# cover-vla/cover-vla

Measured on AMD Instinct MI355X. Metric: candidate actions scored/sec (whole node), OpenVLA-7B N=32, 224^2 RGB, higher is better.
Workload: dtype bf16; 1 GPU; OpenVLA-7B (DINOv2-L+SigLIP-So400m+Llama-2-7B) N=32 = 8 prompts x 4 samples per GPU, 7 action tokens, 1 224x224 RGB frame(s); CoVer verifier SigLIP2-L/16-384 + 3-member ensemble; random-init weights with decision margins (depth-scaled residual projections, unit-scale embeddings, log-normal gains on the action rows of the head: synth.openvla_state(peaked=True)); candidates_total=32, candidates_per_gpu=32, prompts_per_gpu=8, parallelism=candidate-sharded x1 (weak), own_kv=legacy

## Files before the change

### cover_vla_amd/_lib.py

```python
from __future__ import annotations

import ctypes as C
import os

import torch

_HERE = os.path.dirname(os.path.abspath(__file__))
LIB_PATH = os.environ.get("COVER_LIB_PATH") or os.path.join(_HERE, "libcover_hip.so")

c_p = C.c_void_p
c_ll = C.c_longlong
c_i = C.c_int
c_f = C.c_float


class CoverError(RuntimeError):
    pass


class GemmEpi(C.Structure):
    _fields_ = [("bias", c_p), ("residual", c_p), ("layer_scale", c_p), ("ld_residual", c_i), ("residual_f32", c_i),
                ("act", c_i), ("glu", c_i), ("out_f32", c_i), ("out_scale", c_f),
                ("norm_w", c_p), ("norm_out", c_p), ("ld_norm_out", c_i), ("norm_style", c_i), ("norm_w_offset", c_f),
                ("norm_eps", c_f), ("norm_b", c_p), ("w8", c_p), ("w8_scale", c_p), ("a8", c_p), ("a8_scale", c_p), ("ld_a8", c_i), ("ld_norm_out8", c_i),
                ("norm_out8", c_p), ("norm_out8_scale", c_p),
                ("a8_mx", c_p), ("out8", c_p), ("out8_mx", c_p), ("ld_out8", c_i), ("w8_klinear", c_i)]


class KvSegment(C.Structure):
    _fields_ = [("k", c_p), ("vt", c_p),
                ("k_slot_stride", c_ll), ("k_t_stride", c_ll), ("k_h_stride", c_ll),
                ("vt_slot_stride", c_ll), ("vt_h_stride", c_ll), ("vt_d_stride", c_ll),
                ("slot_of_batch", c_p), ("len_of_batch", c_p), ("vis_len", c_p),
                ("len", c_i), ("mask_mode", c_i), ("causal_offset", c_i), ("_pad", c_i)]


class AttnArgs(C.Structure):
    _fields_ = [("q", c_p), ("out", c_p),
                ("q_b_stride", c_ll), ("q_t_stride", c_ll), ("q_h_stride", c_ll),
                ("o_b_stride", c_ll), ("o_t_stride", c_ll), ("o_h_stride", c_ll),
                ("B", c_i), ("Tq", c_i), ("Hq", c_i), ("Hkv", c_i), ("D", c_i), ("scale", c_f),
                ("n_seg", c_i), ("_pad", c_i), ("seg", KvSegment * 3),
                ("state_in_o", c_p), ("state_in_ml", c_p), ("state_out_o", c_p), ("state_out_ml", c_p),
                ("out8", c_p), ("out8_mx", c_p), ("out8_rows", c_i), ("_pad2", c_i)]


class DecodeAttnArgs(C.Structure):
    _fields_ = [("qkv", c_p), ("ld_qkv", c_i), ("n_splits", c_i), ("partial", c_p), ("bias", c_p),
                ("N", c_i), ("H", c_i), ("D", c_i), ("scale", c_f),
                ("positions", c_p), ("cos_table", c_p), ("sin_table", c_p), ("n_pos", c_i), ("rope_mode", c_i),
                ("seg", KvSegment * 3), ("write_t", c_i), ("_pad", c_i), ("out", c_p), ("out_row_stride", c_ll)]


class OwnAttnArgs(C.Structure):
    _fields_ = [("qkv", c_p), ("ld_qkv", c_i), ("N", c_i), ("H", c_i), ("D", c_i), ("scale", c_f),
                ("positions", c_p), ("cos_table", c_p), ("sin_table", c_p), ("n_pos", c_i), ("rope_mode", c_i),
                ("k", c_p), ("v", c_p), ("k_scale", c_p), ("v_scale", c_p), ("fp8", c_i), ("t_cap", c_i),
                ("slot_stride", c_ll), ("slot_of_batch", c_p), ("write_t", c_i), ("_pad", c_i),
                ("state_o", c_p), ("state_ml", c_p)]


class RopeArgs(C.Structure):
    _fields_ = [("qkv", c_p), ("ld_qkv", c_i),
                ("B", c_i), ("T", c_i), ("Hq", c_i), ("Hkv", c_i), ("D", c_i),
                ("positions", c_p), ("cos_table", c_p), ("sin_table", c_p), ("n_pos", c_i),
                ("rope_mode", c_i),
                ("k_cache", c_p), ("k_slot_stride", c_ll), ("k_t_stride", c_ll), ("k_h_stride", c_ll),
# ... 297 lines not shown
```

### cover_vla_amd/csrc/attention.hip

```cpp
#include <stdlib.h>
#include <string.h>
#include "common.h"
#include "kernels.h"

struct SegDev {
    const bf16_t* k;
    const bf16_t* vt;
    long long k_slot, k_t, k_h, vt_slot, vt_h, vt_d;
    const int* slot_of_batch;
    const int* len_of_batch;
    const int* vis_len;
    int len, mode, causal_off;
};
struct AttnDev {
    const bf16_t* q;
    bf16_t* out;
    long long q_b, q_t, q_h, o_b, o_t, o_h;
    int B, Tq, Hq, Hkv, G, R;
    float scale_log2e;
    int n_seg;
    SegDev seg[3];
    const float* si_o; const float* si_ml;
    float* so_o; float* so_ml;
    uint8_t* o8; uint8_t* o8mx; int o8_rows;
    bool shared;
};

#ifdef COVER_AT_DEBUG
__device__ unsigned long long g_at_dbg[512 * 8];
extern "C" int cover_at_debug(unsigned long long* out) { return (int)hipMemcpyFromSymbol(out, HIP_SYMBOL(g_at_dbg), sizeof(g_at_dbg)); }
#define ATT(slot) do { if (threadIdx.x == 0) g_at_dbg[(((blockIdx.z * gridDim.y + blockIdx.y) * gridDim.x + blockIdx.x) & 511) * 8 + (slot)] = wall_clock64(); } while (0)
#else
#define ATT(slot) do { } while (0)
#endif
template <int D, bool KSPLIT, int NWS = 4, bool MXO = false>
__device__ __forceinline__ void attn_body(const AttnDev& a, int bx, int kvh, int b) {
    ATT(0);
    constexpr int KS = D / 32;
    constexpr int DB = D / 16;
    static_assert(!MXO || (KSPLIT && DB == 2 * NWS), "block-scaled output: two adjacent d blocks per wave");
    extern __shared__ __attribute__((aligned(16))) char smem[];
    const int lane = threadIdx.x & 63;
    const int w = __builtin_amdgcn_readfirstlane(threadIdx.x >> 6);
    const int nw = KSPLIT ? NWS : (int)(blockDim.x >> 6);
    const int tile = KSPLIT ? bx : bx * nw + w;
    const int r = lane & 15, g = lane >> 4;

    const int qi = tile * 16 + r;
    const bool q_ok = qi < a.R;
    const int qc = q_ok ? qi : 0;
    const int t = qc / a.G, gh = qc - t * a.G;
    const int h = kvh * a.G + gh;
    if (!KSPLIT && tile * 16 >= a.R) return;

    bf16x8 qf[KS];
    {
        const bf16_t* qp = a.q + (long long)b * a.q_b + (long long)t * a.q_t + (long long)h * a.q_h + g * 8;
#pragma unroll
        for (int ks = 0; ks < KS; ++ks) qf[ks] = as_bf16x8(*(const uint4*)(qp + ks * 32));
    }

#ifdef COVER_AT_DEBUG
    asm volatile("s_waitcnt vmcnt(0)" ::: "memory");
    ATT(1);
#endif
    float m_run = -INFINITY, l_run = 0.f;
    f32x4 oacc[DB];
#pragma unroll
    for (int db = 0; db < DB; ++db) oacc[db] = (f32x4){0.f, 0.f, 0.f, 0.f};
    const long long srow = ((long long)b * a.Tq + t) * a.Hq + h;
    if (a.si_o && q_ok && (!KSPLIT || w == 0)) {
        m_run = a.si_ml[srow * 2];
        l_run = a.si_ml[srow * 2 + 1];
        const float* so = a.si_o + srow * D + 4 * g;
#pragma unroll
        for (int db = 0; db < DB; ++db) {
            const float4 v = *(const float4*)(so + db * 16);
            oacc[db] = (f32x4){v.x * l_run, v.y * l_run, v.z * l_run, v.w * l_run};
        }
    }

    int t_hi = (tile * 16 + 15) / a.G;
    t_hi = t_hi < a.Tq ? t_hi : a.Tq - 1;

    int tile_counter = 0;
    for (int si = 0; si < a.n_seg; ++si) {
        const SegDev& sg = a.seg[si];
        const int slot = sg.slot_of_batch ? sg.slot_of_batch[b] : b;
        const int len = sg.len_of_batch ? sg.len_of_batch[b] : sg.len;
        int kend = len;
        if (sg.mode == COVER_MASK_CAUSAL) kend = min(kend, t_hi + sg.causal_off + 1);
        int vis = len;
        if (sg.mode == COVER_MASK_CAUSAL) vis = min(len, t + sg.causal_off + 1);
        else if (sg.mode == COVER_MASK_VISLEN) vis = min(len, sg.vis_len[t]);
        const bf16_t* kb = sg.k + (long long)slot * sg.k_slot + (long long)kvh * sg.k_h + g * 8;
        const bf16_t* vb = sg.vt + (long long)slot * sg.vt_slot + (long long)kvh * sg.vt_h + (long long)r * sg.vt_d + g * 8;

        for (int t0 = 0; t0 < kend; t0 += 32, ++tile_counter) {
            if (KSPLIT && (tile_counter & (nw - 1)) != w) continue;
            int key0 = t0 + 8 * (r >> 2) + (r & 3);
            int key1 = key0 + 4;
            key0 = key0 < len ? key0 : len - 1;
            key1 = key1 < len ? key1 : len - 1;
            const bf16_t* k0p = kb + (long long)key0 * sg.k_t;
            const bf16_t* k1p = kb + (long long)key1 * sg.k_t;
            const bf16_t* vp = vb + t0;
            uint4 kr0[KS], kr1[KS];
#pragma unroll
            for (int ks = 0; ks < KS; ++ks) {
                kr0[ks] = *(const uint4*)(k0p + ks * 32);
                kr1[ks] = *(const uint4*)(k1p + ks * 32);
            }
            constexpr bool V_EARLY = (D <= 128) || KSPLIT;
            uint4 vr[V_EARLY ? DB : 1];
            if (V_EARLY) {
#pragma unroll
                for (int db = 0; db < DB; ++db) vr[db] = *(const uint4*)(vp + (long long)(db * 16) * sg.vt_d);
            }
#ifdef COVER_AT_DEBUG
            if (tile_counter == 0) { asm volatile("s_waitcnt vmcnt(0)" ::: "memory"); ATT(2); }
#endif
            f32x4 s0 = (f32x4){0.f, 0.f, 0.f, 0.f}, s1 = s0;
#pragma unroll
            for (int ks = 0; ks < KS; ++ks) {
                s0 = __builtin_amdgcn_mfma_f32_16x16x32_bf16(as_bf16x8(kr0[ks]), qf[ks], s0, 0, 0, 0);
                s1 = __builtin_amdgcn_mfma_f32_16x16x32_bf16(as_bf16x8(kr1[ks]), qf[ks], s1, 0, 0, 0);
            }
            float sc[8];
            float tmax = -INFINITY;
#pragma unroll
            for (int e = 0; e < 8; ++e) {
                const float v = (e < 4 ? s0[e] : s1[e - 4]) * a.scale_log2e;
                const int key = t0 + 8 * g + e;
                sc[e] = (key < vis) ? v : -INFINITY;
                tmax = fmaxf(tmax, sc[e]);
            }
            tmax = fmaxf(tmax, __shfl_xor(tmax, 16));
            tmax = fmaxf(tmax, __shfl_xor(tmax, 32));
            const float m_new = fmaxf(m_run, tmax);
            float alpha = 1.f, psum = 0.f;
            float p[8];
            if (m_new == -INFINITY) {
#pragma unroll
                for (int e = 0; e < 8; ++e) p[e] = 0.f;
            } else {
                alpha = exp2f(m_run - m_new);
#pragma unroll
                for (int e = 0; e < 8; ++e) {
                    p[e] = exp2f(sc[e] - m_new);
                    psum += p[e];
                }
            }
            psum += __shfl_xor(psum, 16);
            psum += __shfl_xor(psum, 32);
            l_run = l_run * alpha + psum;
            m_run = m_new;
            uint4 pp;
            pp.x = pack_bf2(p[0], p[1]);
            pp.y = pack_bf2(p[2], p[3]);
            pp.z = pack_bf2(p[4], p[5]);
            pp.w = pack_bf2(p[6], p[7]);
            const bf16x8 pf = as_bf16x8(pp);
#pragma unroll
            for (int db = 0; db < DB; ++db) {
                const bf16x8 vf = as_bf16x8(V_EARLY ? vr[V_EARLY ? db : 0] : *(const uint4*)(vp + (long long)(db * 16) * sg.vt_d));
                f32x4 o = oacc[db];
                o[0] *= alpha; o[1] *= alpha; o[2] *= alpha; o[3] *= alpha;
                oacc[db] = __builtin_amdgcn_mfma_f32_16x16x32_bf16(vf, pf, o, 0, 0, 0);
            }
        }
    }

    ATT(3);
    int db_first = 0, db_step = 1;
    if (KSPLIT) {
        float* so = (float*)smem;
        constexpr int OW = DB * 4 * 64;
        float* sm = so + NWS * OW;
        float* sl = sm + NWS * 16;
#pragma unroll
        for (int db = 0; db < DB; ++db)
#pragma unroll
            for (int e = 0; e < 4; ++e) so[w * OW + (db * 4 + e) * 64 + lane] = oacc[db][e];
        if (g == 0) {
            sm[w * 16 + r] = m_run;
            sl[w * 16 + r] = l_run;
        }
        __syncthreads();
        float mi[NWS], li[NWS], f[NWS];
#pragma unroll
        for (int i = 0; i < NWS; ++i) {
            mi[i] = sm[i * 16 + r];
            li[i] = sl[i * 16 + r];
        }
        float mx = -INFINITY;
#pragma unroll
        for (int i = 0; i < NWS; ++i) mx = fmaxf(mx, mi[i]);
        float lt = 0.f;
// ... 315 lines not shown
            const float is = 1.0f / scl;
            const int col = h * (int)a.o_h + 32 * j;
#pragma unroll
            for (int k = 0; k < 2; ++k) {
                int pk = __builtin_amdgcn_cvt_pk_fp8_f32(v[k * 4] * is, v[k * 4 + 1] * is, 0, false);
                pk = __builtin_amdgcn_cvt_pk_fp8_f32(v[k * 4 + 2] * is, v[k * 4 + 3] * is, pk, true);
                *(uint32_t*)(a.o8 + ro + col + k * 16 + 4 * g) = (uint32_t)pk;
            }
            if (g == 0) a.o8mx[((size_t)(col >> 7) * a.o8_rows + (size_t)(ro / a.o_t)) * 4 + ((col >> 5) & 3)] = (uint8_t)((__builtin_bit_cast(uint32_t, scl) >> 23) & 0xffu);
        }
        ATT(5);
        return;
    }
    if (a.so_o) {
        if (g == 0) {
            a.so_ml[srow * 2] = m_run;
            a.so_ml[srow * 2 + 1] = l_run;
        }
        float* so = a.so_o + srow * D + 4 * g;
#pragma unroll
        for (int db = 0; db < DB; ++db) *(float4*)(so + db * 16) = make_float4(oacc[db][0] * inv, oacc[db][1] * inv, oacc[db][2] * inv, oacc[db][3] * inv);
        return;
    }
    bf16_t* op = a.out + (long long)b * a.o_b + (long long)t * a.o_t + (long long)h * a.o_h + 4 * g;
#pragma unroll
    for (int db = 0; db < DB; ++db) {
        uint2 v;
        v.x = pack_bf2(oacc[db][0] * inv, oacc[db][1] * inv);
        v.y = pack_bf2(oacc[db][2] * inv, oacc[db][3] * inv);
        *(uint2*)(op + db * 16) = v;
    }
    ATT(5);
}
template <int D, bool KSPLIT, int NWS = 4, bool MXO = false>
__global__ __launch_bounds__((KSPLIT && D > 128) ? 64 * NWS : 512) void attn_kernel(AttnDev a) {
    attn_body<D, KSPLIT, NWS, MXO>(a, blockIdx.x, blockIdx.y, blockIdx.z);
}
template <int D>
__global__ __launch_bounds__(512) void attn_kernel_dual(AttnDev a0, AttnDev a1, int tiles0, int n0, int tiles1) {
    int idx = blockIdx.x;
    if (idx < n0) {
        attn_body<D, true>(a0, idx % tiles0, blockIdx.y, idx / tiles0);
    } else {
        idx -= n0;
        attn_body<D, true>(a1, idx % tiles1, blockIdx.y, idx / tiles1);
    }
}

struct AttnEnv {
    bool shared_off, pair_off, has_ks_max;
    long long ks_max, nw8_max;
};
static const AttnEnv& attn_env() {
    static const AttnEnv e = [] {
        AttnEnv v;
        const char* sh = getenv("COVER_ATTN_SHARED");
        const char* pr = getenv("COVER_ATTN_PAIR");
        const char* mx = getenv("COVER_ATTN_KSPLIT_MAX");
        const char* n8 = getenv("COVER_ATTN_NW8_MAX");
        v.shared_off = sh && sh[0] == '0';
        v.pair_off = pr && pr[0] == '0';
        v.has_ks_max = mx != nullptr;
        v.ks_max = mx ? atoll(mx) : 1023;
        v.nw8_max = n8 ? atoll(n8) : 0;
        return v;
    }();
    return e;
}
static long long attn_qtiles(const cover_attn_args* x) {
    const int G = x->Hq / x->Hkv;
    return (long long)((x->Tq * G + 15) / 16) * x->Hkv * x->B;
}
static long long attn_ks_max(const cover_attn_args* x) {
    const AttnEnv& e = attn_env();
    return (x->state_in_o != nullptr && !e.has_ks_max && x->D <= 128) ? 4095 : e.ks_max;
}
static bool attn_shared_ok(const cover_attn_args* x) {
    if (attn_env().shared_off) return false;
    if (x->D != 128 || x->Hq != x->Hkv || x->Tq < 48 || x->n_seg < 1 || x->n_seg > 3) return false;
    for (int i = 0; i < x->n_seg; ++i)
        if (x->seg[i].mask_mode != COVER_MASK_LEN) return false;
    return (long long)((x->Tq + 63) / 64) * x->Hq * x->B >= 128;
}

bool attention_mx_ok(const cover_attn_args* x) {
    if (x->D != 128 || x->Hq != x->Hkv || x->Hkv <= 0 || x->state_out_o != nullptr || x->B <= 0 || x->Tq <= 0) return false;
    if (x->o_h_stride != 128 || x->o_t_stride != (long long)x->Hq * 128 || (x->o_b_stride % x->o_t_stride) != 0) return false;
    return attn_qtiles(x) <= attn_ks_max(x) || attn_shared_ok(x);
}

struct AttnPlan {
    int form, mxo, nw;
    dim3 grid;
    size_t lds;
};
static hipError_t attn_decide(const cover_attn_args* x, AttnPlan& p) {
    p.form = -1; p.mxo = 0; p.nw = 0; p.grid = dim3(0, 0, 0); p.lds = 0;
    const int G = x->Hq / x->Hkv, R = x->Tq * G;
    if (x->B <= 0 || R <= 0) return hipSuccess;
    const int D = x->D;
    if (D != 64 && D != 96 && D != 128 && D != 256) return hipErrorInvalidValue;
    const bool o8 = x->out8 != nullptr && x->out8_mx != nullptr;
    const int tiles = (R + 15) / 16;
    const long long qtiles = (long long)tiles * x->Hkv * x->B;
    const long long ks_max = attn_ks_max(x);
    p.mxo = o8 ? 1 : 0;
    if (attn_shared_ok(x)) {
        p.form = 3; p.nw = 4;
        p.grid = dim3((x->Tq + 63) / 64, x->Hq, x->B);
        return hipSuccess;
    }
    if (o8) {
        if (D != 128 || qtiles > ks_max) return hipErrorInvalidValue;
        p.form = 1; p.nw = 4;
    } else if (qtiles <= ks_max) {
        p.nw = (qtiles <= attn_env().nw8_max && D <= 128) ? 8 : 4;
        p.form = p.nw == 8 ? 2 : 1;
    } else {
        p.form = 0;
        p.nw = tiles >= 4 ? 4 : tiles;
        p.grid = dim3((tiles + p.nw - 1) / p.nw, x->Hkv, x->B);
        return hipSuccess;
    }
    p.grid = dim3(tiles, x->Hkv, x->B);
    p.lds = (size_t)(p.nw * (D / 16) * 4 * 64 + 2 * p.nw * 16) * sizeof(float);
    return hipSuccess;
}
static bool attn_pair_dual(const cover_attn_args* x0, const cover_attn_args* x1) {
    const AttnEnv& e = attn_env();
    const bool o8 = (x0->out8 && x0->out8_mx) || (x1->out8 && x1->out8_mx);
    return x0->D == x1->D && x0->Hkv == x1->Hkv && x0->B > 0 && x1->B > 0 && x0->Tq > 0 && x1->Tq > 0 && attn_qtiles(x0) <= e.ks_max &&
           attn_qtiles(x1) <= e.ks_max && (x0->D == 64 || x0->D == 96 || x0->D == 128) && !o8 && !e.pair_off;
}

static bool off16(const void* p) { return ((uintptr_t)p & 15) != 0; }
static hipError_t build_attn_dev(const cover_attn_args* x, AttnDev& a) {
    if (x->n_seg < 1 || x->n_seg > 3 || x->Hkv <= 0 || x->Hq % x->Hkv != 0) return hipErrorInvalidValue;
    a.q = (const bf16_t*)x->q;
    a.out = (bf16_t*)x->out;
    a.q_b = x->q_b_stride; a.q_t = x->q_t_stride; a.q_h = x->q_h_stride;
    a.o_b = x->o_b_stride; a.o_t = x->o_t_stride; a.o_h = x->o_h_stride;
    if (off16(a.q) || ((a.q_b | a.q_t | a.q_h) & 7)) return hipErrorInvalidValue;
    if (((uintptr_t)a.out & 7) || ((a.o_b | a.o_t | a.o_h) & 3)) return hipErrorInvalidValue;
    a.B = x->B; a.Tq = x->Tq; a.Hq = x->Hq; a.Hkv = x->Hkv;
    a.G = x->Hq / x->Hkv;
    a.R = x->Tq * a.G;
    a.scale_log2e = x->scale * 1.4426950408889634f;
    a.n_seg = x->n_seg;
    a.si_o = x->state_in_o; a.si_ml = x->state_in_ml; a.so_o = x->state_out_o; a.so_ml = x->state_out_ml;
    if ((a.si_o == nullptr) != (a.si_ml == nullptr) || (a.so_o == nullptr) != (a.so_ml == nullptr)) return hipErrorInvalidValue;
    if (off16(a.si_o) || off16(a.so_o) || ((uintptr_t)a.si_ml & 7) || ((uintptr_t)a.so_ml & 7)) return hipErrorInvalidValue;
    a.o8 = (uint8_t*)x->out8; a.o8mx = (uint8_t*)x->out8_mx; a.o8_rows = x->out8_rows;
    if (!a.o8 || !a.o8mx) { a.o8 = nullptr; a.o8mx = nullptr; }
    if (a.o8 && !attention_mx_ok(x)) return hipErrorInvalidValue;
    a.shared = attn_shared_ok(x);
    for (int i = 0; i < x->n_seg; ++i) {
        const cover_kv_segment& s = x->seg[i];
        SegDev& d = a.seg[i];
        d.k = (const bf16_t*)s.k; d.vt = (const bf16_t*)s.vt;
        d.k_slot = s.k_slot_stride; d.k_t = s.k_t_stride; d.k_h = s.k_h_stride;
        d.vt_slot = s.vt_slot_stride; d.vt_h = s.vt_h_stride; d.vt_d = s.vt_d_stride;
        d.slot_of_batch = s.slot_of_batch; d.len_of_batch = s.len_of_batch; d.vis_len = s.vis_len;
        d.len = s.len; d.mode = s.mask_mode; d.causal_off = s.causal_offset;
        if (d.mode == COVER_MASK_VISLEN && d.vis_len == nullptr) return hipErrorInvalidValue;
        if (off16(d.k) || off16(d.vt) || ((d.k_slot | d.k_t | d.k_h | d.vt_slot | d.vt_h | d.vt_d) & 7)) return hipErrorInvalidValue;
    }
    return hipSuccess;
}

hipError_t attention_plan(const cover_attn_args* x, int* plan) {
    AttnDev a;
    AttnPlan p;
    hipError_t e = build_attn_dev(x, a);
    if (e == hipSuccess) e = attn_decide(x, p);
    if (e != hipSuccess) return e;
    plan[0] = p.form; plan[1] = p.mxo; plan[2] = (int)(p.grid.x * p.grid.y * p.grid.z); plan[3] = p.nw;
    return hipSuccess;
}
hipError_t attention_pair_plan(const cover_attn_args* x0, const cover_attn_args* x1, int* dual) {
    AttnDev a;
    AttnPlan p;
    hipError_t e = build_attn_dev(x0, a);
    if (e == hipSuccess) e = attn_decide(x0, p);
    if (e == hipSuccess) e = build_attn_dev(x1, a);
    if (e == hipSuccess) e = attn_decide(x1, p);
    if (e != hipSuccess) return e;
    *dual = attn_pair_dual(x0, x1) ? 1 : 0;
    return hipSuccess;
}

template <int D>
static void launch_d(const AttnDev& a, const AttnPlan& p, hipStream_t st) {
    const dim3 block(64 * p.nw);
    if (p.form == 3) {
        if (p.mxo) hipLaunchKernelGGL((attn_shared_k<true>), p.grid, block, 0, st, a);
        else hipLaunchKernelGGL((attn_shared_k<false>), p.grid, block, 0, st, a);
    } else if (p.form == 1 && p.mxo) {
        if constexpr (D == 128) hipLaunchKernelGGL((attn_kernel<D, true, 4, true>), p.grid, block, p.lds, st, a);
    } else if (p.form == 2) {
        if constexpr (D <= 128) hipLaunchKernelGGL((attn_kernel<D, true, 8>), p.grid, block, p.lds, st, a);
    } else if (p.form == 1) {
        hipLaunchKernelGGL((attn_kernel<D, true, 4>), p.grid, block, p.lds, st, a);
    } else {
        hipLaunchKernelGGL((attn_kernel<D, false>), p.grid, block, 0, st, a);
    }
}
static hipError_t launch_planned(const cover_attn_args* x, const AttnDev& a, const AttnPlan& p, hipStream_t st) {
    if (p.form < 0) return hipSuccess;
    const int pid = prof_enabled() ? prof_open(st, 2, 0.0) : -1;
    switch (x->D) {
        case 64: launch_d<64>(a, p, st); break;
        case 96: launch_d<96>(a, p, st); break;
        case 128: launch_d<128>(a, p, st); break;
        default: launch_d<256>(a, p, st); break;
    }
    const hipError_t e = hipGetLastError();
    prof_close(st, pid);
    return e;
}

hipError_t launch_attention_bf16(const cover_attn_args* x, hipStream_t st) {
    AttnDev a;
    AttnPlan p;
    hipError_t e = build_attn_dev(x, a);
    if (e == hipSuccess) e = attn_decide(x, p);
    if (e != hipSuccess) return e;
    return launch_planned(x, a, p, st);
// ... 33 lines not shown
```

### cover_vla_amd/csrc/capi.hip

```cpp
#include <hip/hip_runtime.h>
#include <stdio.h>
#include <stdlib.h>
#include <string.h>
#include <string>
#include "kernels.h"

static thread_local std::string g_err;
static int fail(int code, const char* what, hipError_t e = hipSuccess) {
    char buf[512];
    if (e != hipSuccess) snprintf(buf, sizeof buf, "%s: %s", what, hipGetErrorString(e));
    else snprintf(buf, sizeof buf, "%s", what);
    g_err = buf;
    return code;
}
#define HIPCHK(call, what)                                  \
    do {                                                    \
        hipError_t _e = (call);                             \
        if (_e != hipSuccess) return fail(_e == hipErrorInvalidValue ? COVER_EINVAL : COVER_EHIP, what, _e); \
    } while (0)
#define ST(s) ((hipStream_t)(s))

extern "C" {

int cover_abi_version(void) { return COVER_ABI_VERSION; }
// ... 426 lines not shown
    size_t skb = 0;
    {
        const int ns[4] = {3 * HD, d->dim, d->mlp_p, d->dim};
        const int ks[4] = {d->dim, HD, d->dim, d->mlp_p};
        for (int i = 0; i < 4; ++i) {
            size_t b = gemm_workspace_bytes((int)R, ns[i], ks[i]);
            skb = b > skb ? b : skb;
        }
    }
    p = cc.take(skb); if (sk) *sk = p;
    if (sk_bytes) *sk_bytes = skb;
    return cc.off + 256;
}
size_t cover_vit_workspace_bytes(const cover_vit_desc* d, int n_seq, int T) {
    int tcap;
    return vit_ws(d, n_seq, T, nullptr, nullptr, nullptr, nullptr, nullptr, nullptr, nullptr, nullptr, &tcap);
}

__global__ void zero_u32_k(unsigned* __restrict__ p, size_t n) {
    for (size_t i = (size_t)blockIdx.x * blockDim.x + threadIdx.x; i < n; i += (size_t)gridDim.x * blockDim.x) p[i] = 0u;
}
int cover_vit_forward(const cover_vit_desc* d, void* x, int n_seq, int T, void* attn_out, cover_workspace ws, int variant,
                      void* stream) {
    if (!d || !x || !d->layers_host) return fail(COVER_EINVAL, "cover_vit_forward: null pointer");
    if (d->last_attn_only && !attn_out) return fail(COVER_EINVAL, "cover_vit_forward: last_attn_only needs attn_out");
    hipStream_t st = ST(stream);
    Carver c{(char*)ws.ptr, ws.bytes, 0};
    void *h, *qkv, *attn, *mlp, *vt, *sk;
    size_t skb;
    int tcap;
    const size_t need = vit_ws(d, n_seq, T, &c, &h, &qkv, &attn, &mlp, &vt, &sk, &skb, &tcap);
    if (!ws.ptr || ws.bytes < need) return fail(COVER_EWORKSPACE, "cover_vit_forward: workspace too small");
    const int R = n_seq * T, dim = d->dim, H = d->heads, Dp = d->head_dim_p, HD = H * Dp;
    if (tcap != T) {
        const size_t words = (size_t)n_seq * HD * tcap / 2;
        hipLaunchKernelGGL(zero_u32_k, dim3((unsigned)((words + 1023) / 1024 < 2048 ? (words + 1023) / 1024 : 2048)), dim3(256), 0, st, (unsigned*)vt, words);
        HIPCHK(hipGetLastError(), "zero vt");
    }

    HIPCHK(launch_layernorm_bf16((const bf16_t*)x, dim, d->layers_host[0].ln1_w, d->layers_host[0].ln1_b, (bf16_t*)h, dim, R, dim, d->ln_eps, st), "vit ln1");
    for (int l = 0; l < d->n_layers; ++l) {
        const cover_vit_layer& L = d->layers_host[l];
        cover_gemm_epi e;
        memset(&e, 0, sizeof e);
        e.out_scale = 1.0f;
        e.bias = L.qkv_b;
        HIPCHK(launch_gemm_bf16((const bf16_t*)h, dim, (const bf16_t*)L.qkv_w, qkv, 3 * HD, R, 3 * HD, dim, &e, (float*)sk, skb, variant, st), "vit qkv");
        cover_rope_args ra;
        memset(&ra, 0, sizeof ra);
        ra.qkv = qkv; ra.ld_qkv = 3 * HD; ra.B = n_seq; ra.T = T; ra.Hq = H; ra.Hkv = H; ra.D = Dp; ra.rope_mode = 0;
        ra.vt_cache = vt; ra.vt_slot_stride = (long long)HD * tcap; ra.vt_h_stride = (long long)Dp * tcap; ra.vt_d_stride = tcap;
        HIPCHK(launch_rope_kv_write(&ra, st), "vit v-transpose");
        cover_attn_args aa;
        memset(&aa, 0, sizeof aa);
        aa.q = qkv; aa.q_b_stride = (long long)T * 3 * HD; aa.q_t_stride = 3 * HD; aa.q_h_stride = Dp;
        aa.out = attn; aa.o_b_stride = (long long)T * HD; aa.o_t_stride = HD; aa.o_h_stride = Dp;
        aa.B = n_seq; aa.Tq = T; aa.Hq = H; aa.Hkv = H; aa.D = Dp; aa.scale = d->attn_scale; aa.n_seg = 1;
        aa.seg[0].k = (const bf16_t*)qkv + HD; aa.seg[0].k_slot_stride = (long long)T * 3 * HD; aa.seg[0].k_t_stride = 3 * HD; aa.seg[0].k_h_stride = Dp;
        aa.seg[0].vt = vt; aa.seg[0].vt_slot_stride = (long long)HD * tcap; aa.seg[0].vt_h_stride = (long long)Dp * tcap; aa.seg[0].vt_d_stride = tcap;
        aa.seg[0].len = T; aa.seg[0].mask_mode = COVER_MASK_LEN;
        HIPCHK(launch_attention_bf16(&aa, st), "vit attention");
        const bool last_attn = d->last_attn_only && l == d->n_layers - 1;
        memset(&e, 0, sizeof e);
        e.out_scale = 1.0f;
        e.bias = L.proj_b;
        if (last_attn) {
            HIPCHK(launch_gemm_bf16((const bf16_t*)attn, HD, (const bf16_t*)L.proj_w, attn_out, dim, R, dim, HD, &e, (float*)sk, skb, variant, st), "vit proj (tap)");
            break;
        }
        e.residual = x; e.ld_residual = dim; e.layer_scale = L.ls1;
        e.norm_w = L.ln2_w; e.norm_b = L.ln2_b; e.norm_out = h; e.ld_norm_out = dim; e.norm_style = 2; e.norm_eps = d->ln_eps;
        HIPCHK(launch_gemm_bf16((const bf16_t*)attn, HD, (const bf16_t*)L.proj_w, x, dim, R, dim, HD, &e, (float*)sk, skb, variant, st), "vit proj (+ln2)");
        memset(&e, 0, sizeof e);
        e.out_scale = 1.0f;
        e.bias = L.fc1_b; e.act = d->act;
        HIPCHK(launch_gemm_bf16((const bf16_t*)h, dim, (const bf16_t*)L.fc1_w, mlp, d->mlp_p, R, d->mlp_p, dim, &e, (float*)sk, skb, variant, st), "vit fc1");
        memset(&e, 0, sizeof e);
        e.out_scale = 1.0f;
        e.bias = L.fc2_b; e.residual = x; e.ld_residual = dim; e.layer_scale = L.ls2;
        if (l + 1 < d->n_layers) {
            const cover_vit_layer& Ln = d->layers_host[l + 1];
            e.norm_w = Ln.ln1_w; e.norm_b = Ln.ln1_b; e.norm_out = h; e.ld_norm_out = dim; e.norm_style = 2; e.norm_eps = d->ln_eps;
        }
        HIPCHK(launch_gemm_bf16((const bf16_t*)mlp, d->mlp_p, (const bf16_t*)L.fc2_w, x, dim, R, dim, d->mlp_p, &e, (float*)sk, skb, variant, st), "vit fc2 (+next ln1)");
    }
    return COVER_OK;
}

static size_t dec_ws(const cover_dec_desc* d, int rows, Carver* c, void** h, void** qkv, void** attn, void** mlp, void** sk,
                     size_t* sk_bytes, void** st_o = nullptr, void** st_ml = nullptr, void** q8 = nullptr, void** q8s = nullptr, void** q8mx = nullptr) {
    Carver tmp{nullptr, 0, 0};
    Carver& cc = c ? *c : tmp;
    const int nqkv = (d->Hq + 2 * d->Hkv) * d->D;
// ... 336 lines not shown
```

### cover_vla_amd/ops.py

```python
from __future__ import annotations

import ctypes as C
import math
from dataclasses import dataclass
from typing import Optional, Sequence, Union

import numpy as np
import torch

from . import _lib as L

ACT = {"none": 0, "gelu_tanh": 1, "gelu_erf": 2, "silu": 3, "relu": 4}
MASK_LEN, MASK_CAUSAL, MASK_VISLEN = 0, 1, 2


def _stream() -> int:
    return torch.cuda.current_stream().cuda_stream


def _ptr(t: Optional[torch.Tensor]) -> Optional[int]:
    return None if t is None else t.data_ptr()


def _chk_dev(*ts):
# ... 136 lines not shown
    torch.cuda.synchronize()
    buf = (C.c_ulonglong * 16)()
    L.check(L.lib().cover_gemm_probe(buf), "gemm_probe")
    w0, w1, w2, w3, c0, c1, nk = (int(buf[i]) for i in range(7))
    e4, e5, e6 = (int(buf[i]) for i in (12, 13, 14))
    loop_us = (w2 - w1) * 0.01
    staged = w2 <= e4 <= e5 <= e6 <= w3
    return dict(prologue_us=(w1 - w0) * 0.01, loop_us=loop_us, epilogue_us=(w3 - w2) * 0.01, k_tiles=nk,
                cycles_per_k_tile=(c1 - c0) / max(nk, 1), clock_ghz=(c1 - c0) / max(loop_us, 1e-9) / 1e3,
                epilogue_split_us=[(e4 - w2) * 0.01, (e5 - e4) * 0.01, (e6 - e5) * 0.01, (w3 - e6) * 0.01] if staged else None)


def gemm_plan_counts(reset: bool = False) -> list:
    n = 32
    buf = (C.c_longlong * n)()
    L.lib().cover_gemm_plan_counts(buf, n, 1 if reset else 0)
    return list(buf)


@dataclass
class Segment:
    k: torch.Tensor
    vt: torch.Tensor
    k_strides: Sequence[int]
    vt_strides: Sequence[int]
    length: int = 0
    len_of_batch: Optional[torch.Tensor] = None
    slot_of_batch: Optional[torch.Tensor] = None
    mask: int = MASK_LEN
    causal_offset: int = 0
    vis_len: Optional[torch.Tensor] = None
    k_offset: int = 0
    vt_offset: int = 0


def fill_segment(s: L.KvSegment, seg: Segment) -> None:
    s.k = seg.k.data_ptr() + 2 * seg.k_offset
    s.vt = seg.vt.data_ptr() + 2 * seg.vt_offset
    s.k_slot_stride, s.k_t_stride, s.k_h_stride = seg.k_strides
    s.vt_slot_stride, s.vt_h_stride, s.vt_d_stride = seg.vt_strides
    s.slot_of_batch = _ptr(seg.slot_of_batch)
    s.len_of_batch = _ptr(seg.len_of_batch)
    s.vis_len = _ptr(seg.vis_len)
    s.len = seg.length
    s.mask_mode = seg.mask
    s.causal_offset = seg.causal_offset


def attention_args(q: torch.Tensor, q_strides: Sequence[int], out: Optional[torch.Tensor], o_strides: Sequence[int], B: int, Tq: int,
                   Hq: int, Hkv: int, D: int, scale: float, segments: Sequence[Segment], state_in=None, state_out=None, out8=None) -> "L.AttnArgs":
    _chk_dev(q, out)
    a = L.AttnArgs()
    a._keep = (q, out, out8, state_in, state_out, list(segments))
    a.q, a.out = q.data_ptr(), _ptr(out)
    if out8 is not None:
        _chk_dev(out8[0], out8[1])
        assert out8[0].dtype == torch.uint8 and out8[1].dtype == torch.uint8 and out8[1].is_contiguous() and out8[0].is_contiguous()
        a.out8, a.out8_mx, a.out8_rows = out8[0].data_ptr(), out8[1].data_ptr(), out8[0].shape[0]
    if state_in is not None:
        a.state_in_o, a.state_in_ml = state_in[0].data_ptr(), state_in[1].data_ptr()
    if state_out is not None:
        a.state_out_o, a.state_out_ml = state_out[0].data_ptr(), state_out[1].data_ptr()
    a.q_b_stride, a.q_t_stride, a.q_h_stride = q_strides
    a.o_b_stride, a.o_t_stride, a.o_h_stride = o_strides
    a.B, a.Tq, a.Hq, a.Hkv, a.D, a.scale = B, Tq, Hq, Hkv, D, scale
    a.n_seg = len(segments)
    for i, sg in enumerate(segments[:3]):
        fill_segment(a.seg[i], sg)
    return a
# ... 997 lines not shown
```

### include/cover_hip.h

```cpp
#ifndef COVER_HIP_H
#define COVER_HIP_H
#include <stddef.h>
#include <stdint.h>

#ifdef __cplusplus
extern "C" {
#endif

#define COVER_ABI_VERSION 1

enum cover_status { COVER_OK = 0, COVER_EINVAL = -1, COVER_EHIP = -2, COVER_EWORKSPACE = -3, COVER_EUNSUPPORTED = -4 };
enum cover_act { COVER_ACT_NONE = 0, COVER_ACT_GELU_TANH = 1, COVER_ACT_GELU_ERF = 2, COVER_ACT_SILU = 3, COVER_ACT_RELU = 4 };

int cover_abi_version(void);
const char* cover_last_error(void);
int cover_device_info(int dev, int* n_cu, size_t* total_mem, char* name, int name_len);

typedef struct cover_gemm_epi {
    const float* bias;
    const void* residual;
    const float* layer_scale;
    int ld_residual;
    int residual_f32;
    int act;
// ... 25 lines not shown
size_t cover_packed_weight_bytes(int N, int K);
int cover_packed_k(int K);
int cover_pack_weight_bf16(const void* W, int ldw, int N, int K, void* Wp, int glu_interleave, void* stream);

size_t cover_packed_weight_fp8_bytes(int N, int K);
int cover_quantize_rows_fp8(const void* W, int ldw, int N, int K, float* scales, void* Wdq, void* stream);
int cover_pack_weight_fp8(const void* Wdq, int ldw, const float* scales, int N, int K, void* Wq, float* scales_packed,
                          int glu_interleave, void* stream);

int cover_quantize_act_fp8(const void* X, int ldx, int M, int K, void* out8, int ld8, float* scales, void* stream);
int cover_quantize_act_fp8_mx(const void* X, int ldx, int M, int K, void* out8, int ld8, void* mx, void* stream);
int cover_pack_weight_fp8_klinear(const void* Wdq, int ldw, const float* scales, int N, int K, void* Wq, float* scales_packed, void* stream);

size_t cover_gemm_workspace_bytes(int M, int N, int K);
int cover_gemm_bf16(const void* A, int lda, const void* Wp, void* C, int ldc, int M, int N, int K,
                    const cover_gemm_epi* epi, void* splitk_ws, size_t splitk_ws_bytes, int variant, void* stream);
int cover_gemm_plan_counts(long long* counts, int n, int reset);
int cover_gemm_plan(const void* A, int lda, const void* Wp, void* C, int ldc, int M, int N, int K,
                    const cover_gemm_epi* epi, void* splitk_ws, size_t splitk_ws_bytes, int variant, int plan[6]);
int cover_gemm_probe(unsigned long long* out);

enum cover_mask_mode { COVER_MASK_LEN = 0, COVER_MASK_CAUSAL = 1, COVER_MASK_VISLEN = 2 };
typedef struct cover_kv_segment {
    const void* k;
    const void* vt;
    long long k_slot_stride, k_t_stride, k_h_stride;
    long long vt_slot_stride, vt_h_stride, vt_d_stride;
    const int* slot_of_batch;
    const int* len_of_batch;
    const int* vis_len;
    int len;
    int mask_mode;
    int causal_offset;
    int _pad;
} cover_kv_segment;

typedef struct cover_attn_args {
    const void* q;
    void* out;
    long long q_b_stride, q_t_stride, q_h_stride;
    long long o_b_stride, o_t_stride, o_h_stride;
    int B, Tq, Hq, Hkv, D;
    float scale;
    int n_seg;
    int _pad;
    cover_kv_segment seg[3];
    const float* state_in_o; const float* state_in_ml;
    float* state_out_o; float* state_out_ml;
    void* out8; void* out8_mx;
    int out8_rows; int _pad2;
} cover_attn_args;
int cover_attention_bf16(const cover_attn_args* args, void* stream);
int cover_attention_plan(const cover_attn_args* args, int plan[4]);
int cover_attention_bf16_pair(const cover_attn_args* a0, const cover_attn_args* a1, void* stream);
int cover_attention_pair_plan(const cover_attn_args* a0, const cover_attn_args* a1, int* dual);

typedef struct cover_decode_attn_args {
    const void* qkv; int ld_qkv;
    int n_splits;
    const float* partial; const float* bias;
    int N, H, D;
    float scale;
    const int* positions; const float* cos_table; const float* sin_table; int n_pos; int rope_mode;
    cover_kv_segment seg[3];
    int write_t; int _pad;
    void* out; long long out_row_stride;
} cover_decode_attn_args;
// ... 270 lines not shown
    const float* logprobs;
    long long lp_n_stride, lp_t_stride;
    const int64_t* tokens;
    long long tok_n_stride, tok_t_stride;
    long long pad_token_id;
    int N, steps, group_size, top_m;
    float beta; int length_normalize;
    float* prior_out;
    float* combined_out;
    float* group_mean_out;
    int* result_out;
    float* best_out;
    int* ranked_out;
} cover_prior_select_args;
int cover_prior_select(const cover_prior_select_args* args, void* stream);

typedef struct cover_workspace { void* ptr; size_t bytes; } cover_workspace;

typedef struct cover_vit_layer {
    const float *ln1_w, *ln1_b, *ln2_w, *ln2_b;
    const void* qkv_w; const float* qkv_b;
    const void* proj_w; const float* proj_b;
    const void* fc1_w; const float* fc1_b;
    const void* fc2_w; const float* fc2_b;
    const float *ls1, *ls2;
} cover_vit_layer;
typedef struct cover_vit_desc {
    int dim, heads, head_dim_p, mlp_p, n_layers, act;
    float ln_eps, attn_scale;
    const cover_vit_layer* layers_host;
    int last_attn_only;
    int _pad;
} cover_vit_desc;
size_t cover_vit_workspace_bytes(const cover_vit_desc* d, int n_seq, int T);
int cover_vit_forward(const cover_vit_desc* d, void* x, int n_seq, int T, void* attn_out, cover_workspace ws,
                      int gemm_variant, void* stream);

typedef struct cover_dec_layer {
    const float* in_norm_w; const float* post_norm_w;
    const void* qkv_w; const float* qkv_b;
    const void* o_w;
    const void* gate_up_w;
    const void* down_w;
    void* k_cache; void* vt_cache;
    const void* qkv_w8; const float* qkv_s; const void* o_w8; const float* o_s;
    const void* gate_up_w8; const float* gate_up_s; const void* down_w8; const float* down_s;
    int down_klinear;
    int o_klinear;
} cover_dec_layer;
typedef struct cover_dec_desc {
    int dim, Hq, Hkv, D, mlp, n_layers, act;
    int norm_style;
    float norm_eps, norm_w_offset, attn_scale;
    int rope_mode; int n_pos; int _pad;
    const float* cos_table; const float* sin_table;
    const float* final_norm_w;
    const cover_dec_layer* layers_host;
} cover_dec_desc;
typedef struct cover_dec_group {
    int B, T;
    const int* positions;
    int n_seg; int write_seg;
    cover_kv_segment segs[3];
    long long seg_k_offset[3], seg_vt_offset[3];
    const int* write_slot_of_batch; const int* write_t_offset_of_batch;
    int write_t_offset;
// ... 45 lines not shown
```

Baseline: 951.8 candidates/s.

## Read row-major V directly in ViT attention via LDS transpose reads

Adds a row-major V path to the attention kernel for head sizes 64 and 96. V rows are loaded straight from the packed QKV buffer, staged in swizzled LDS, and transposed with ds_read_tr16_b64 to form the MFMA operand. The ViT forward now uses this path by default, which removes the separate per-layer V-transpose kernel and its global-memory round trip. The cost is extra LDS per wave and an LDS write/read per KV tile, and the path turns off dual-pair launches. An environment variable or variant flag restores the old transpose path.

```diff
diff --git a/cover_vla_amd/_lib.py b/cover_vla_amd/_lib.py
--- a/cover_vla_amd/_lib.py
+++ b/cover_vla_amd/_lib.py
@@ -32,7 +32,7 @@
                 ("k_slot_stride", c_ll), ("k_t_stride", c_ll), ("k_h_stride", c_ll),
                 ("vt_slot_stride", c_ll), ("vt_h_stride", c_ll), ("vt_d_stride", c_ll),
                 ("slot_of_batch", c_p), ("len_of_batch", c_p), ("vis_len", c_p),
-                ("len", c_i), ("mask_mode", c_i), ("causal_offset", c_i), ("_pad", c_i)]
+                ("len", c_i), ("mask_mode", c_i), ("causal_offset", c_i), ("v_rowmajor", c_i)]
 
 
 class AttnArgs(C.Structure):
diff --git a/cover_vla_amd/csrc/attention.hip b/cover_vla_amd/csrc/attention.hip
--- a/cover_vla_amd/csrc/attention.hip
+++ b/cover_vla_amd/csrc/attention.hip
@@ -24,7 +24,17 @@
     float* so_o; float* so_ml;
     uint8_t* o8; uint8_t* o8mx; int o8_rows;
     bool shared;
+    bool vrow;
 };
+
+template <int D> struct VRowStage {
+    static constexpr int PITCH = D == 64 ? 128 : 256;
+    static constexpr int BYTES = 32 * PITCH;
+};
+template <int D> __device__ __forceinline__ int vrow_swz(int row) {
+    return D == 64 ? (((row >> 1) & 1) | (((row >> 3) & 1) << 1)) : ((row & 3) | (((row >> 3) & 1) << 2));
+}
+typedef short vrow_s4 __attribute__((ext_vector_type(4)));
 
 #ifdef COVER_AT_DEBUG
 __device__ unsigned long long g_at_dbg[512 * 8];
@@ -33,12 +43,13 @@
 #else
 #define ATT(slot) do { } while (0)
 #endif
-template <int D, bool KSPLIT, int NWS = 4, bool MXO = false>
+template <int D, bool KSPLIT, int NWS = 4, bool MXO = false, bool VROW = false>
 __device__ __forceinline__ void attn_body(const AttnDev& a, int bx, int kvh, int b) {
     ATT(0);
     constexpr int KS = D / 32;
     constexpr int DB = D / 16;
     static_assert(!MXO || (KSPLIT && DB == 2 * NWS), "block-scaled output: two adjacent d blocks per wave");
+    static_assert(!VROW || ((D == 64 || D == 96) && !MXO), "row-major V: the tower head sizes");
     extern __shared__ __attribute__((aligned(16))) char smem[];
     const int lane = threadIdx.x & 63;
     const int w = __builtin_amdgcn_readfirstlane(threadIdx.x >> 6);
@@ -94,7 +105,7 @@
         if (sg.mode == COVER_MASK_CAUSAL) vis = min(len, t + sg.causal_off + 1);
         else if (sg.mode == COVER_MASK_VISLEN) vis = min(len, sg.vis_len[t]);
         const bf16_t* kb = sg.k + (long long)slot * sg.k_slot + (long long)kvh * sg.k_h + g * 8;
-        const bf16_t* vb = sg.vt + (long long)slot * sg.vt_slot + (long long)kvh * sg.vt_h + (long long)r * sg.vt_d + g * 8;
+        const bf16_t* vb = sg.vt + (long long)slot * sg.vt_slot + (long long)kvh * sg.vt_h + (VROW ? (long long)((lane & 1) * 8) : (long long)r * sg.vt_d + g * 8);
 
         for (int t0 = 0; t0 < kend; t0 += 32, ++tile_counter) {
             if (KSPLIT && (tile_counter & (nw - 1)) != w) continue;
@@ -113,7 +124,13 @@
             }
             constexpr bool V_EARLY = (D <= 128) || KSPLIT;
             uint4 vr[V_EARLY ? DB : 1];
-            if (V_EARLY) {
+            if constexpr (VROW) {
+                int vkey = t0 + (lane >> 1);
+                vkey = vkey < len ? vkey : len - 1;
+                const bf16_t* vrp = vb + (long long)vkey * sg.vt_d;
+#pragma unroll
+                for (int db = 0; db < DB; ++db) vr[db] = *(const uint4*)(vrp + db * 16);
+            } else if (V_EARLY) {
 #pragma unroll
                 for (int db = 0; db < DB; ++db) vr[db] = *(const uint4*)(vp + (long long)(db * 16) * sg.vt_d);
             }
@@ -161,9 +178,34 @@
             pp.z = pack_bf2(p[4], p[5]);
             pp.w = pack_bf2(p[6], p[7]);
             const bf16x8 pf = as_bf16x8(pp);
+            if constexpr (VROW) {
+                if (t0 + 32 > len && t0 + (lane >> 1) >= len) {
+#pragma unroll
+                    for (int db = 0; db < DB; ++db) vr[db] = make_uint4(0u, 0u, 0u, 0u);
+                }
+                using VS = VRowStage<D>;
+                char* vst = smem + (KSPLIT ? (NWS * DB * 4 * 64 + 2 * NWS * 16) * (int)sizeof(float) : 0) + w * VS::BYTES;
+                char* vwr = vst + (lane >> 1) * VS::PITCH + (lane & 1) * 16;
+                const int sw = vrow_swz<D>(lane >> 1);
+#pragma unroll
+                for (int db = 0; db < DB; ++db) *(uint4*)(vwr + ((db ^ sw) << 5)) = vr[db];
+                const char* vrd = vst + (8 * g + (r >> 2)) * VS::PITCH + (r & 3) * 8;
+                const int sr = vrow_swz<D>(8 * g + (r >> 2));
+#pragma unroll
+                for (int db = 0; db < DB; ++db) {
+                    const vrow_s4 lo = __builtin_amdgcn_ds_read_tr16_b64_v4i16((__attribute__((address_space(3))) vrow_s4*)(vrd + ((db ^ sr) << 5)));
+                    const vrow_s4 hi = __builtin_amdgcn_ds_read_tr16_b64_v4i16((__attribute__((address_space(3))) vrow_s4*)(vrd + 4 * VS::PITCH + ((db ^ sr) << 5)));
+                    uint4 u;
+                    u.x = ((uint32_t)(uint16_t)lo[0]) | ((uint32_t)(uint16_t)lo[1] << 16);
+                    u.y = ((uint32_t)(uint16_t)lo[2]) | ((uint32_t)(uint16_t)lo[3] << 16);
+                    u.z = ((uint32_t)(uint16_t)hi[0]) | ((uint32_t)(uint16_t)hi[1] << 16);
+                    u.w = ((uint32_t)(uint16_t)hi[2]) | ((uint32_t)(uint16_t)hi[3] << 16);
+                    vr[db] = u;
+                }
+            }
 #pragma unroll
             for (int db = 0; db < DB; ++db) {
-                const bf16x8 vf = as_bf16x8(V_EARLY ? vr[V_EARLY ? db : 0] : *(const uint4*)(vp + (long long)(db * 16) * sg.vt_d));
+                const bf16x8 vf = as_bf16x8((V_EARLY || VROW) ? vr[(V_EARLY || VROW) ? db : 0] : *(const uint4*)(vp + (long long)(db * 16) * sg.vt_d));
                 f32x4 o = oacc[db];
                 o[0] *= alpha; o[1] *= alpha; o[2] *= alpha; o[3] *= alpha;
                 oacc[db] = __builtin_amdgcn_mfma_f32_16x16x32_bf16(vf, pf, o, 0, 0, 0);
@@ -545,9 +587,9 @@
     }
     ATT(5);
 }
-template <int D, bool KSPLIT, int NWS = 4, bool MXO = false>
+template <int D, bool KSPLIT, int NWS = 4, bool MXO = false, bool VROW = false>
 __global__ __launch_bounds__((KSPLIT && D > 128) ? 64 * NWS : 512) void attn_kernel(AttnDev a) {
-    attn_body<D, KSPLIT, NWS, MXO>(a, blockIdx.x, blockIdx.y, blockIdx.z);
+    attn_body<D, KSPLIT, NWS, MXO, VROW>(a, blockIdx.x, blockIdx.y, blockIdx.z);
 }
 template <int D>
 __global__ __launch_bounds__(512) void attn_kernel_dual(AttnDev a0, AttnDev a1, int tiles0, int n0, int tiles1) {
@@ -607,7 +649,23 @@
     dim3 grid;
     size_t lds;
 };
+static hipError_t attn_decide_form(const cover_attn_args* x, AttnPlan& p);
+static bool attn_vrow(const cover_attn_args* x) {
+    for (int i = 0; i < x->n_seg && i < 3; ++i)
+        if (x->seg[i].v_rowmajor != 0) return true;
+    return false;
+}
 static hipError_t attn_decide(const cover_attn_args* x, AttnPlan& p) {
+    const hipError_t e = attn_decide_form(x, p);
+    if (e != hipSuccess || !attn_vrow(x)) return e;
+    if (x->n_seg != 1 || x->seg[0].v_rowmajor != 1 || x->seg[0].mask_mode != COVER_MASK_LEN || (x->D != 64 && x->D != 96)) return hipErrorInvalidValue;
+    if ((x->out8 && x->out8_mx) || x->state_in_o || x->state_out_o) return hipErrorInvalidValue;
+    if (p.form < 0) return hipSuccess;
+    if (p.form != 0 && p.form != 1) return hipErrorInvalidValue;
+    p.lds += (size_t)p.nw * (x->D == 64 ? VRowStage<64>::BYTES : VRowStage<96>::BYTES);
+    return hipSuccess;
+}
+static hipError_t attn_decide_form(const cover_attn_args* x, AttnPlan& p) {
     p.form = -1; p.mxo = 0; p.nw = 0; p.grid = dim3(0, 0, 0); p.lds = 0;
     const int G = x->Hq / x->Hkv, R = x->Tq * G;
     if (x->B <= 0 || R <= 0) return hipSuccess;
@@ -642,6 +700,7 @@
 static bool attn_pair_dual(const cover_attn_args* x0, const cover_attn_args* x1) {
     const AttnEnv& e = attn_env();
     const bool o8 = (x0->out8 && x0->out8_mx) || (x1->out8 && x1->out8_mx);
+    if (attn_vrow(x0) || attn_vrow(x1)) return false;
     return x0->D == x1->D && x0->Hkv == x1->Hkv && x0->B > 0 && x1->B > 0 && x0->Tq > 0 && x1->Tq > 0 && attn_qtiles(x0) <= e.ks_max &&
            attn_qtiles(x1) <= e.ks_max && (x0->D == 64 || x0->D == 96 || x0->D == 128) && !o8 && !e.pair_off;
 }
@@ -667,9 +726,11 @@
     if (!a.o8 || !a.o8mx) { a.o8 = nullptr; a.o8mx = nullptr; }
     if (a.o8 && !attention_mx_ok(x)) return hipErrorInvalidValue;
     a.shared = attn_shared_ok(x);
+    a.vrow = attn_vrow(x);
     for (int i = 0; i < x->n_seg; ++i) {
         const cover_kv_segment& s = x->seg[i];
         SegDev& d = a.seg[i];
+        if (s.v_rowmajor != 0 && s.v_rowmajor != 1) return hipErrorInvalidValue;
         d.k = (const bf16_t*)s.k; d.vt = (const bf16_t*)s.vt;
         d.k_slot = s.k_slot_stride; d.k_t = s.k_t_stride; d.k_h = s.k_h_stride;
         d.vt_slot = s.vt_slot_stride; d.vt_h = s.vt_h_stride; d.vt_d = s.vt_d_stride;
@@ -705,7 +766,12 @@
 template <int D>
 static void launch_d(const AttnDev& a, const AttnPlan& p, hipStream_t st) {
     const dim3 block(64 * p.nw);
-    if (p.form == 3) {
+    if (a.vrow) {
+        if constexpr (D == 64 || D == 96) {
+            if (p.form == 1) hipLaunchKernelGGL((attn_kernel<D, true, 4, false, true>), p.grid, block, p.lds, st, a);
+            else hipLaunchKernelGGL((attn_kernel<D, false, 4, false, true>), p.grid, block, p.lds, st, a);
+        }
+    } else if (p.form == 3) {
         if (p.mxo) hipLaunchKernelGGL((attn_shared_k<true>), p.grid, block, 0, st, a);
         else hipLaunchKernelGGL((attn_shared_k<false>), p.grid, block, 0, st, a);
     } else if (p.form == 1 && p.mxo) {
diff --git a/cover_vla_amd/csrc/capi.hip b/cover_vla_amd/csrc/capi.hip
--- a/cover_vla_amd/csrc/capi.hip
+++ b/cover_vla_amd/csrc/capi.hip
@@ -482,7 +482,27 @@
     const size_t need = vit_ws(d, n_seq, T, &c, &h, &qkv, &attn, &mlp, &vt, &sk, &skb, &tcap);
     if (!ws.ptr || ws.bytes < need) return fail(COVER_EWORKSPACE, "cover_vit_forward: workspace too small");
     const int R = n_seq * T, dim = d->dim, H = d->heads, Dp = d->head_dim_p, HD = H * Dp;
-    if (tcap != T) {
+    static const bool vt_env = [] { const char* v = getenv("COVER_VIT_V_TRANSPOSE"); return v && v[0] == '1'; }();
+    cover_attn_args aa;
+    memset(&aa, 0, sizeof aa);
+    aa.q = qkv; aa.q_b_stride = (long long)T * 3 * HD; aa.q_t_stride = 3 * HD; aa.q_h_stride = Dp;
+    aa.out = attn; aa.o_b_stride = (long long)T * HD; aa.o_t_stride = HD; aa.o_h_stride = Dp;
+    aa.B = n_seq; aa.Tq = T; aa.Hq = H; aa.Hkv = H; aa.D = Dp; aa.scale = d->attn_scale; aa.n_seg = 1;
+    aa.seg[0].k = (const bf16_t*)qkv + HD; aa.seg[0].k_slot_stride = (long long)T * 3 * HD; aa.seg[0].k_t_stride = 3 * HD; aa.seg[0].k_h_stride = Dp;
+    aa.seg[0].vt = (const bf16_t*)qkv + 2 * HD; aa.seg[0].vt_slot_stride = (long long)T * 3 * HD; aa.seg[0].vt_h_stride = Dp; aa.seg[0].vt_d_stride = 3 * HD;
+    aa.seg[0].v_rowmajor = 1;
+    aa.seg[0].len = T; aa.seg[0].mask_mode = COVER_MASK_LEN;
+    bool v_transpose = vt_env || (variant & COVER_VIT_V_TRANSPOSE) != 0;
+    variant &= 0xff;
+    if (!v_transpose) {
+        int plan[4];
+        v_transpose = attention_plan(&aa, plan) != hipSuccess;
+    }
+    if (v_transpose) {
+        aa.seg[0].vt = vt; aa.seg[0].vt_slot_stride = (long long)HD * tcap; aa.seg[0].vt_h_stride = (long long)Dp * tcap; aa.seg[0].vt_d_stride = tcap;
+        aa.seg[0].v_rowmajor = 0;
+    }
+    if (v_transpose && tcap != T) {
         const size_t words = (size_t)n_seq * HD * tcap / 2;
         hipLaunchKernelGGL(zero_u32_k, dim3((unsigned)((words + 1023) / 1024 < 2048 ? (words + 1023) / 1024 : 2048)), dim3(256), 0, st, (unsigned*)vt, words);
         HIPCHK(hipGetLastError(), "zero vt");
@@ -496,19 +516,13 @@
         e.out_scale = 1.0f;
         e.bias = L.qkv_b;
         HIPCHK(launch_gemm_bf16((const bf16_t*)h, dim, (const bf16_t*)L.qkv_w, qkv, 3 * HD, R, 3 * HD, dim, &e, (float*)sk, skb, variant, st), "vit qkv");
-        cover_rope_args ra;
-        memset(&ra, 0, sizeof ra);
-        ra.qkv = qkv; ra.ld_qkv = 3 * HD; ra.B = n_seq; ra.T = T; ra.Hq = H; ra.Hkv = H; ra.D = Dp; ra.rope_mode = 0;
-        ra.vt_cache = vt; ra.vt_slot_stride = (long long)HD * tcap; ra.vt_h_stride = (long long)Dp * tcap; ra.vt_d_stride = tcap;
-        HIPCHK(launch_rope_kv_write(&ra, st), "vit v-transpose");
-        cover_attn_args aa;
-        memset(&aa, 0, sizeof aa);
-        aa.q = qkv; aa.q_b_stride = (long long)T * 3 * HD; aa.q_t_stride = 3 * HD; aa.q_h_stride = Dp;
-        aa.out = attn; aa.o_b_stride = (long long)T * HD; aa.o_t_stride = HD; aa.o_h_stride = Dp;
-        aa.B = n_seq; aa.Tq = T; aa.Hq = H; aa.Hkv = H; aa.D = Dp; aa.scale = d->attn_scale; aa.n_seg = 1;
-        aa.seg[0].k = (const bf16_t*)qkv + HD; aa.seg[0].k_slot_stride = (long long)T * 3 * HD; aa.seg[0].k_t_stride = 3 * HD; aa.seg[0].k_h_stride = Dp;
-        aa.seg[0].vt = vt; aa.seg[0].vt_slot_stride = (long long)HD * tcap; aa.seg[0].vt_h_stride = (long long)Dp * tcap; aa.seg[0].vt_d_stride = tcap;
-        aa.seg[0].len = T; aa.seg[0].mask_mode = COVER_MASK_LEN;
+        if (v_transpose) {
+            cover_rope_args ra;
+            memset(&ra, 0, sizeof ra);
+            ra.qkv = qkv; ra.ld_qkv = 3 * HD; ra.B = n_seq; ra.T = T; ra.Hq = H; ra.Hkv = H; ra.D = Dp; ra.rope_mode = 0;
+            ra.vt_cache = vt; ra.vt_slot_stride = (long long)HD * tcap; ra.vt_h_stride = (long long)Dp * tcap; ra.vt_d_stride = tcap;
+            HIPCHK(launch_rope_kv_write(&ra, st), "vit v-transpose");
+        }
         HIPCHK(launch_attention_bf16(&aa, st), "vit attention");
         const bool last_attn = d->last_attn_only && l == d->n_layers - 1;
         memset(&e, 0, sizeof e);
diff --git a/cover_vla_amd/ops.py b/cover_vla_amd/ops.py
--- a/cover_vla_amd/ops.py
+++ b/cover_vla_amd/ops.py
@@ -192,9 +192,11 @@
     vis_len: Optional[torch.Tensor] = None
     k_offset: int = 0
     vt_offset: int = 0
+    v_rowmajor: bool = False
 
 
 def fill_segment(s: L.KvSegment, seg: Segment) -> None:
+    s.v_rowmajor = 1 if seg.v_rowmajor else 0
     s.k = seg.k.data_ptr() + 2 * seg.k_offset
     s.vt = seg.vt.data_ptr() + 2 * seg.vt_offset
     s.k_slot_stride, s.k_t_stride, s.k_h_stride = seg.k_strides
diff --git a/include/cover_hip.h b/include/cover_hip.h
--- a/include/cover_hip.h
+++ b/include/cover_hip.h
@@ -81,7 +81,7 @@
     int len;
     int mask_mode;
     int causal_offset;
-    int _pad;
+    int v_rowmajor;
 } cover_kv_segment;
 
 typedef struct cover_attn_args {
@@ -418,6 +418,7 @@
     int last_attn_only;
     int _pad;
 } cover_vit_desc;
+#define COVER_VIT_V_TRANSPOSE 0x100
 size_t cover_vit_workspace_bytes(const cover_vit_desc* d, int n_seq, int T);
 int cover_vit_forward(const cover_vit_desc* d, void* x, int n_seq, int T, void* attn_out, cover_workspace ws,
                       int gemm_variant, void* stream);
```

Result: no change. 949.7 candidates/s (-0.2%).
